# yzhang511/multi_modal_foundation_model

Hardware: AMD Instinct MI355X
Metric: pretrain samples/sec (T=100 bins/modality, d_model=256, 5+5 layers, spike+behaviour masked pretraining step) (higher is better)
Workload: dtype bf16; 1 GPU; BASELINE.json configs[1]: 1 session, ap(668 neurons)+behaviour(2), d_model=256, heads=8, mlp=512, 5 enc + 5 dec layers, T=100 (L=200 tokens), dropout 0.4/0.2, AdamW+OneCycleLR, mixed objectives; per_gpu_batch=1024, global_batch=1024, seq_len=200, parallelism=dp1

## Files before the change

multi_modal_foundation_model_amd/csrc/gemm_bf16.hip:

```cpp
#include "gemm_route.h"
#include <stdlib.h>
#include <algorithm>

namespace {

constexpr int BM = 128, BN = 128;
constexpr int NTHREADS = 256;
template <int BK> struct Geo {
    static constexpr int KC_LD = BK + 8;
    static constexpr int TILE_BYTES = 128 * KC_LD * 2;
    static constexpr int NP = BK / 16;
};

typedef __attribute__((ext_vector_type(8))) __bf16 bf16x8v;
typedef __attribute__((ext_vector_type(4))) short s16x4;
typedef __attribute__((address_space(3))) s16x4 lds_s16x4;

__device__ __forceinline__ uint4 load8(const uint16_t* __restrict__ src, int nvalid, int align) {
    uint4 v = make_uint4(0u, 0u, 0u, 0u);
    if (nvalid >= 8 && align == 8) return *reinterpret_cast<const uint4*>(src);
    if (nvalid >= 8 && align == 4) {
        const uint2 a = *reinterpret_cast<const uint2*>(src), b = *reinterpret_cast<const uint2*>(src + 4);
        return make_uint4(a.x, a.y, b.x, b.y);
    }
    if (nvalid <= 0) return v;
    uint16_t e[8];
#pragma unroll
    for (int j = 0; j < 8; ++j) e[j] = (j < nvalid) ? src[j] : (uint16_t)0;
    v.x = e[0] | ((uint32_t)e[1] << 16); v.y = e[2] | ((uint32_t)e[3] << 16);
    v.z = e[4] | ((uint32_t)e[5] << 16); v.w = e[6] | ((uint32_t)e[7] << 16);
    return v;
}

template <bool RC, int BK>
__device__ __forceinline__ void g2r(uint4 (&r)[BK / 16], const uint16_t* __restrict__ base, int ld, int row0, int k0, int rows, int kend,
                                    int align, int t) {
    constexpr int NP = BK / 16, LPR = BK / 8, RPP = 256 / LPR;
    if (!RC) {
        const int kq = t % LPR, r0 = t / LPR, k = k0 + 8 * kq;
#pragma unroll
        for (int p = 0; p < NP; ++p) {
            const int row = row0 + r0 + RPP * p;
            r[p] = (row < rows) ? load8(base + (size_t)row * ld + k, kend - k, align) : make_uint4(0u, 0u, 0u, 0u);
        }
    } else {
        const int cq = t & 15, kk0 = t >> 4, col = row0 + 8 * cq;
#pragma unroll
        for (int p = 0; p < NP; ++p) {
            const int k = k0 + kk0 + 16 * p;
            r[p] = (k < kend) ? load8(base + (size_t)k * ld + col, rows - col, align) : make_uint4(0u, 0u, 0u, 0u);
        }
    }
}

template <bool RC, int BK>
__device__ __forceinline__ void r2s(char* __restrict__ S, const uint4 (&r)[BK / 16], int t) {
    constexpr int NP = BK / 16, LPR = BK / 8, RPP = 256 / LPR, KC_LD = Geo<BK>::KC_LD;
    if (!RC) {
        const int kq = t % LPR, r0 = t / LPR;
#pragma unroll
        for (int p = 0; p < NP; ++p) *reinterpret_cast<uint4*>(S + (r0 + RPP * p) * (KC_LD * 2) + kq * 16) = r[p];
    } else {
        const int cq = t & 15, kk0 = t >> 4;
#pragma unroll
        for (int p = 0; p < NP; ++p) {
            const int kk = kk0 + 16 * p;
            *reinterpret_cast<uint4*>(S + kk * 256 + ((cq * 16) ^ ((kk & 3) << 6))) = r[p];
        }
    }
}

template <bool RC, int BK>
__device__ __forceinline__ bf16x8v frag(const char* __restrict__ S, int rowbase, int ks, int lane) {
    if (!RC) {
        const int r = lane & 31, h = lane >> 5;
        const uint4 v = *reinterpret_cast<const uint4*>(S + (rowbase + r) * (Geo<BK>::KC_LD * 2) + ks * 32 + h * 16);
        return __builtin_bit_cast(bf16x8v, v);
    } else {
        const int g = lane >> 4, li = lane & 15, q = li >> 2, p = li & 3;
        const int col = rowbase + 16 * (g & 1) + 4 * p;
        const int kb = ks * 16 + 8 * (g >> 1);
        const int off0 = (kb + q) * 256 + ((col * 2) ^ (q << 6));
        const int off1 = (kb + 4 + q) * 256 + ((col * 2) ^ (q << 6));
        const s16x4 lo = __builtin_amdgcn_ds_read_tr16_b64_v4i16((lds_s16x4*)(S + off0));
        const s16x4 hi = __builtin_amdgcn_ds_read_tr16_b64_v4i16((lds_s16x4*)(S + off1));
        typedef __attribute__((ext_vector_type(8))) short s16x8;
        s16x8 v;
        v[0] = lo[0]; v[1] = lo[1]; v[2] = lo[2]; v[3] = lo[3]; v[4] = hi[0]; v[5] = hi[1]; v[6] = hi[2]; v[7] = hi[3];
        return __builtin_bit_cast(bf16x8v, v);
    }
}

template <typename TO, int AK = 0, int EF = 0>
__device__ __forceinline__ void epilogue_store(const mmfm_gemm_desc& d, const LiveArg& lv, const Drop& dr, float v, int m, int n) {
    typedef io<uint16_t> I16;
    constexpr int AKM = AK == kActEmbed ? 0 : AK;
    if (d.bias) v += d.bias[n];
    if (d.pre_out) I16::st(reinterpret_cast<uint16_t*>(d.pre_out) + (size_t)m * d.ldc + n, v);
    if constexpr (AK == kActEmbed) {
        if (!(d.act & 1)) v = embed_act1<true, EF>(v) * d.act_scale;
        else if (EF == 0) v *= d.act_scale;
        else v = embed_mul_grad1<true, EF>(v, I16::ld(reinterpret_cast<const uint16_t*>(d.gradmul_pre) + (size_t)m * d.ldc + n)) * d.act_scale;
        if (dr.on()) v = dr.apply(v, (uint64_t)live_orig_row(lv, m) * (uint64_t)d.N + (uint64_t)n);
        if (d.residual) v += I16::ld(reinterpret_cast<const uint16_t*>(d.residual) + (size_t)m * d.ldr + n);
        io<TO>::st(reinterpret_cast<TO*>(d.C) + (size_t)m * d.ldc + n, v);
        return;
    }
    if (d.act == 1) v = gelu_poly(v);
    else if (d.act == 2) v = softsign_f(v) * d.act_scale;
    else if (AK && !(d.act & 1)) v = mlp_act1<AKM>(v, d.act_scale);
    if (d.gradmul_pre) {
        const float u = I16::ld(reinterpret_cast<const uint16_t*>(d.gradmul_pre) + (size_t)m * d.ldc + n);
        if (AK == MMFM_MLP_RELU) v = u > 0.f ? v : 0.f;
        else if (AK) v *= mlp_act_grad1<AKM>(u, d.act_scale);
        else v *= (d.act == 3) ? gelu_poly_grad(u) : (d.act == 4 ? softsign_grad(u) : softsign_grad_from_out(u, 1.f / d.act_scale)) * d.act_scale;
    }
    if (dr.on()) v = dr.apply(v, (uint64_t)live_orig_row(lv, m) * (uint64_t)d.N + (uint64_t)n);
    if (d.residual) v += I16::ld(reinterpret_cast<const uint16_t*>(d.residual) + (size_t)m * d.ldr + n);
    io<TO>::st(reinterpret_cast<TO*>(d.C) + (size_t)m * d.ldc + n, v);
}

typedef __attribute__((ext_vector_type(8))) __bf16 bf16x8e;
__device__ __forceinline__ bf16x8e pack8f(const float* v) {
    bf16x8e o;
#pragma unroll
    for (int e = 0; e < 8; ++e) o[e] = (__bf16)v[e];
    return o;
}
__device__ __forceinline__ void unpack8(uint4 w, float* u) {
    u[0] = __uint_as_float(w.x << 16); u[1] = __uint_as_float(w.x & 0xffff0000u);
    u[2] = __uint_as_float(w.y << 16); u[3] = __uint_as_float(w.y & 0xffff0000u);
    u[4] = __uint_as_float(w.z << 16); u[5] = __uint_as_float(w.z & 0xffff0000u);
    u[6] = __uint_as_float(w.w << 16); u[7] = __uint_as_float(w.w & 0xffff0000u);
}

__device__ __forceinline__ int xcd_remap(int bid, int nwg) {
    const int q = nwg >> 3, r = nwg & 7, x = bid & 7;
    return (x < r ? x * (q + 1) : r * (q + 1) + (x - r) * q) + (bid >> 3);
}

__device__ __forceinline__ uint4 ldg8(const uint16_t* p, bool a16, bool hi, bool nt) {
    if (a16 && nt) return __builtin_bit_cast(uint4, __builtin_nontemporal_load(reinterpret_cast<const mmfm_u32x4*>(p)));
    if (a16) return *reinterpret_cast<const uint4*>(p);
    const uint2 a = *reinterpret_cast<const uint2*>(p);
    const uint2 b = hi ? *reinterpret_cast<const uint2*>(p + 4) : make_uint2(0u, 0u);
    return make_uint4(a.x, a.y, b.x, b.y);
}
__device__ __forceinline__ void stg8(uint16_t* p, uint4 v, bool a16, bool hi, bool nt) {
    if (nt) {
        if (a16) { st_stream(reinterpret_cast<uint4*>(p), v); return; }
        st_stream(reinterpret_cast<uint2*>(p), make_uint2(v.x, v.y));
        if (hi) st_stream(reinterpret_cast<uint2*>(p + 4), make_uint2(v.z, v.w));
        return;
    }
    if (a16) { *reinterpret_cast<uint4*>(p) = v; return; }
    *reinterpret_cast<uint2*>(p) = make_uint2(v.x, v.y);
    if (hi) *reinterpret_cast<uint2*>(p + 4) = make_uint2(v.z, v.w);
}

template <typename TO, bool EPI_LOADS = true, int AK = 0, int EF = 0>
__device__ __forceinline__ void epilogue_tile(const mmfm_gemm_desc& d, const LiveArg& lv, f32x16 (&acc)[2][2], char* smem, int m0, int n0, int z, int vec_epi,
                                              int t, int wm, int wn, int kh, int l31) {
    const bool split = d.splits > 1;
    constexpr int AKM = AK == kActEmbed ? 0 : AK;
    float* Cf = reinterpret_cast<float*>(d.C) + (split ? (size_t)z * d.slab_stride : 0);
    const Drop dr = drop_init(d.drop);
    if (vec_epi & 1) {
        float* stage = reinterpret_cast<float*>(smem);
        constexpr int SLDW = 132;
        constexpr bool BF_OUT = sizeof(TO) == 2;
        const bool bf_path = BF_OUT && !split;
        const bool a16 = !(vec_epi & 2);
        const int col = (t & 15) * 8, n = n0 + col;
        const bool n_ok = n < d.N, hi = n + 8 <= d.N;
        float bs[8];
#pragma unroll
        for (int e = 0; e < 8; ++e) bs[e] = 0.f;
        if (d.bias && n_ok && !split) {
            const float4 b0 = *reinterpret_cast<const float4*>(d.bias + n);
            const float4 b1 = hi ? *reinterpret_cast<const float4*>(d.bias + n + 4) : make_float4(0.f, 0.f, 0.f, 0.f);
            bs[0] = b0.x; bs[1] = b0.y; bs[2] = b0.z; bs[3] = b0.w; bs[4] = b1.x; bs[5] = b1.y; bs[6] = b1.z; bs[7] = b1.w;
        }
#pragma unroll 1
        for (int half = 0; half < 2; ++half) {
            uint4 gu[4], gr[4];
            if (EPI_LOADS && bf_path) {
#pragma unroll
                for (int c = 0; c < 4; ++c) {
                    const int m = m0 + half * 64 + ((t + 256 * c) >> 4);
                    gu[c] = gr[c] = make_uint4(0u, 0u, 0u, 0u);
                    if (m < d.M && n_ok) {
                        if (d.gradmul_pre) gu[c] = ldg8(reinterpret_cast<const uint16_t*>(d.gradmul_pre) + (size_t)m * d.ldc + n, a16, hi, (vec_epi & 32768) != 0);
                        if (d.residual) gr[c] = ldg8(reinterpret_cast<const uint16_t*>(d.residual) + (size_t)m * d.ldr + n, a16, hi, (vec_epi & 32768) != 0);
                    }
                }
            }
            __syncthreads();
            if (wm == half) {
#pragma unroll
                for (int i = 0; i < 2; ++i)
#pragma unroll
                    for (int j = 0; j < 2; ++j)
#pragma unroll
                        for (int r = 0; r < 16; ++r)
                            stage[(i * 32 + (r & 3) + 8 * (r >> 2) + 4 * kh) * SLDW + wn * 64 + j * 32 + l31] = acc[i][j][r];
            }
            __syncthreads();
#pragma unroll
            for (int c = 0; c < 4; ++c) {
                const int row = (t + 256 * c) >> 4;
                const int m = m0 + half * 64 + row;
                if (m >= d.M || !n_ok) continue;
                float v[8];
                const float4 s0 = *reinterpret_cast<const float4*>(stage + row * SLDW + col);
                const float4 s1 = *reinterpret_cast<const float4*>(stage + row * SLDW + col + 4);
                v[0] = s0.x; v[1] = s0.y; v[2] = s0.z; v[3] = s0.w; v[4] = s1.x; v[5] = s1.y; v[6] = s1.z; v[7] = s1.w;
                const size_t off = (size_t)m * d.ldc + n;
#pragma unroll
                for (int e = 0; e < 8; ++e) v[e] += bs[e];
                if (split || !BF_OUT) {
                    float* dst = (split ? Cf : reinterpret_cast<float*>(d.C)) + off;
                    if (vec_epi & 16384) {
                        st_stream(reinterpret_cast<float4*>(dst), make_float4(v[0], v[1], v[2], v[3]));
                        if (hi) st_stream(reinterpret_cast<float4*>(dst + 4), make_float4(v[4], v[5], v[6], v[7]));
                    } else {
                        *reinterpret_cast<float4*>(dst) = make_float4(v[0], v[1], v[2], v[3]);
                        if (hi) *reinterpret_cast<float4*>(dst + 4) = make_float4(v[4], v[5], v[6], v[7]);
                    }
                    continue;
                }
                if (d.pre_out) stg8(reinterpret_cast<uint16_t*>(d.pre_out) + off, __builtin_bit_cast(uint4, pack8f(v)), a16, hi, (vec_epi & 8192) != 0);
                if constexpr (AK == kActEmbed) {
                    if (!(d.act & 1)) embed_act_n<8, EF>(v, d.act_scale);
                    else {
                        float u[8];
                        unpack8(gu[c], u);
                        embed_mul_grad_n<8, EF>(v, u, d.act_scale);
                    }
                } else if (d.act == 1) gelu_n<8>(v);
                else if (d.act == 2) {
#pragma unroll
                    for (int e = 0; e < 8; ++e) v[e] = softsign_f(v[e]) * d.act_scale;
                } else if (AK && !(d.act & 1)) mlp_act_n<AK, 8>(v, d.act_scale);
                if (AK != kActEmbed && EPI_LOADS && d.gradmul_pre) {
                    float u[8];
                    unpack8(gu[c], u);
                    if (d.act == 3) mul_gelu_grad_n<8>(v, u);
                    else if (d.act == 4) {
#pragma unroll
                        for (int e = 0; e < 8; ++e) v[e] *= softsign_grad(u[e]) * d.act_scale;
                    } else if (AK) mul_mlp_act_grad_n<AKM, 8>(v, u, d.act_scale);
                    else {
                        const float inv_s = 1.f / d.act_scale;
#pragma unroll
                        for (int e = 0; e < 8; ++e) v[e] *= softsign_grad_from_out(u[e], inv_s) * d.act_scale;
                    }
                }
                if (dr.on()) {
                    const uint64_t base = (uint64_t)live_orig_row(lv, m) * (uint64_t)d.N + (uint64_t)n;
#pragma unroll
                    for (int e = 0; e < 8; e += 2) dr.apply2(v[e], v[e + 1], base + e);
                }
                if (EPI_LOADS && d.residual) {
                    float u[8];
                    unpack8(gr[c], u);
#pragma unroll
                    for (int e = 0; e < 8; ++e) v[e] += u[e];
                }
                stg8(reinterpret_cast<uint16_t*>(d.C) + off, __builtin_bit_cast(uint4, pack8f(v)), a16, hi, (vec_epi & 4096) != 0);
            }
        }
        return;
    }
    if (split) {
#pragma unroll
        for (int i = 0; i < 2; ++i)
#pragma unroll
            for (int j = 0; j < 2; ++j)
#pragma unroll
                for (int r = 0; r < 16; ++r) {
                    const int m = m0 + wm * 64 + i * 32 + (r & 3) + 8 * (r >> 2) + 4 * kh;
                    const int n = n0 + wn * 64 + j * 32 + l31;
                    if (m < d.M && n < d.N) Cf[(size_t)m * d.ldc + n] = acc[i][j][r];
                }
        return;
    }
#pragma unroll
    for (int i = 0; i < 2; ++i)
#pragma unroll
        for (int j = 0; j < 2; ++j)
#pragma unroll
            for (int r = 0; r < 16; ++r) {
                const int m = m0 + wm * 64 + i * 32 + (r & 3) + 8 * (r >> 2) + 4 * kh;
                const int n = n0 + wn * 64 + j * 32 + l31;
                if (m < d.M && n < d.N) epilogue_store<TO, AK, EF>(d, lv, dr, acc[i][j][r], m, n);
            }
}

template <bool ARC, bool BRC, typename TO, int BK, bool PERSIST = (sizeof(TO) == 4), int AK = 0>
__global__ __launch_bounds__(NTHREADS, BK == 64 ? 3 : 2) void gemm_bf16_kernel(const mmfm_gemm_desc d_full, const int alignA, const int alignB,
                                                                              const int vec_epi, const int items_full, const LiveArg lv) {
    mmfm_gemm_desc d = d_full;
    live_patch(d, lv);
    const int total_items = (lv.rec && !lv.kdim) ? ((d.M + BM - 1) / BM) * ((d.N + BN - 1) / BN) : items_full;
    constexpr int TILE_BYTES = Geo<BK>::TILE_BYTES;
    __shared__ __attribute__((aligned(16))) char smem[2 * TILE_BYTES];
    char* As = smem;
    char* Bs = smem + TILE_BYTES;
    const int t = threadIdx.x, lane = t & 63, wave = t >> 6;
    const int wm = wave >> 1, wn = wave & 1, kh = lane >> 5, l31 = lane & 31;
    const int tiles_n = (d.N + BN - 1) / BN;
    const int tiles = ((d.M + BM - 1) / BM) * tiles_n;
    const uint16_t* A = reinterpret_cast<const uint16_t*>(d.A);
    const uint16_t* B = reinterpret_cast<const uint16_t*>(d.B);

    auto decode = [&](int w, int& m0, int& n0, int& z, int& kbeg, int& kend) {
        const int item = xcd_remap(w, total_items);
        z = item / tiles;
        const int tile = item - z * tiles;
        m0 = (tile / tiles_n) * BM;
        n0 = (tile % tiles_n) * BN;
        kbeg = z * d.kchunk;
        kend = min(d.K, kbeg + d.kchunk);
    };

    int m0, n0, z, kbeg, kend;
    int w = blockIdx.x;
    if (w >= total_items) return;
    decode(w, m0, n0, z, kbeg, kend);
    uint4 ra[BK / 16], rb[BK / 16];
    g2r<ARC, BK>(ra, A, d.lda, m0, kbeg, d.M, kend, alignA, t);
    g2r<BRC, BK>(rb, B, d.ldb, n0, kbeg, d.N, kend, alignB, t);
    for (;;) {
        f32x16 acc[2][2];
#pragma unroll
        for (int i = 0; i < 2; ++i)
#pragma unroll
            for (int j = 0; j < 2; ++j)
#pragma unroll
                for (int r = 0; r < 16; ++r) acc[i][j][r] = 0.f;
        const bool do_cs = ARC && d.colsum != nullptr && n0 == 0;
        float cs[8];
#pragma unroll
        for (int j = 0; j < 8; ++j) cs[j] = 0.f;
        const int wn_ = w + gridDim.x;
        const bool more = PERSIST && wn_ < total_items;
        int m0n = 0, n0n = 0, zn = 0, kbegn = 0, kendn = 0;
        if (more) decode(wn_, m0n, n0n, zn, kbegn, kendn);
        for (int k0 = kbeg; k0 < kend; k0 += BK) {
            __syncthreads();
            r2s<ARC, BK>(As, ra, t);
            r2s<BRC, BK>(Bs, rb, t);
            __syncthreads();
            {
                if (k0 + BK < kend) {
                    g2r<ARC, BK>(ra, A, d.lda, m0, k0 + BK, d.M, kend, alignA, t);
                    g2r<BRC, BK>(rb, B, d.ldb, n0, k0 + BK, d.N, kend, alignB, t);
                } else if (more) {
                    g2r<ARC, BK>(ra, A, d.lda, m0n, kbegn, d.M, kendn, alignA, t);
                    g2r<BRC, BK>(rb, B, d.ldb, n0n, kbegn, d.N, kendn, alignB, t);
                }
            }
            if (ARC && do_cs) {
                const int cq = t & 15, kk0 = t >> 4;
#pragma unroll
                for (int p = 0; p < BK / 16; ++p) {
                    const int kk = kk0 + 16 * p;
                    float u[8];
                    unpack8(*reinterpret_cast<const uint4*>(As + kk * 256 + ((cq * 16) ^ ((kk & 3) << 6))), u);
#pragma unroll
                    for (int j = 0; j < 8; ++j) cs[j] += u[j];
                }
            }
#pragma unroll
            for (int ks = 0; ks < BK / 16; ++ks) {
                const bf16x8v a0 = frag<ARC, BK>(As, wm * 64, ks, lane), a1 = frag<ARC, BK>(As, wm * 64 + 32, ks, lane);
                const bf16x8v b0 = frag<BRC, BK>(Bs, wn * 64, ks, lane), b1 = frag<BRC, BK>(Bs, wn * 64 + 32, ks, lane);
                acc[0][0] = __builtin_amdgcn_mfma_f32_32x32x16_bf16(a0, b0, acc[0][0], 0, 0, 0);
                acc[0][1] = __builtin_amdgcn_mfma_f32_32x32x16_bf16(a0, b1, acc[0][1], 0, 0, 0);
                acc[1][0] = __builtin_amdgcn_mfma_f32_32x32x16_bf16(a1, b0, acc[1][0], 0, 0, 0);
                acc[1][1] = __builtin_amdgcn_mfma_f32_32x32x16_bf16(a1, b1, acc[1][1], 0, 0, 0);
            }
        }
        if (ARC && do_cs) {
            __syncthreads();
            float* red = reinterpret_cast<float*>(smem);
            float* mine = red + (t >> 4) * 128 + (t & 15) * 8;
            *reinterpret_cast<float4*>(mine) = make_float4(cs[0], cs[1], cs[2], cs[3]);
            *reinterpret_cast<float4*>(mine + 4) = make_float4(cs[4], cs[5], cs[6], cs[7]);
            __syncthreads();
            if (t < 128 && m0 + t < d.M) {
                float sum = 0.f;
#pragma unroll
                for (int i = 0; i < 16; ++i) sum += red[i * 128 + t];
                d.colsum[(d.splits > 1 ? (size_t)z * d.slab_stride : 0) + m0 + t] = sum;
            }
        }
        if constexpr (AK == kActEmbed)
            embed_dispatch(d.act, [&](auto F) {
                epilogue_tile<TO, !(PERSIST && sizeof(TO) == 2), AK, decltype(F)::value>(d, lv, acc, smem, m0, n0, z, vec_epi, t, wm, wn, kh, l31);
            });
        else
            epilogue_tile<TO, !(PERSIST && sizeof(TO) == 2), AK>(d, lv, acc, smem, m0, n0, z, vec_epi, t, wm, wn, kh, l31);
        if (!more) break;
        w = wn_; m0 = m0n; n0 = n0n; z = zn; kbeg = kbegn; kend = kendn;
    }
}

int align_of(const void* p, int ld) {
    if (gemm_ld8(ld) && gemm_al16(p)) return 8;
    if (ld % 4 == 0 && (uintptr_t)p % 8 == 0) return 4;
    return 1;
}

}

int mmfm_gemm_bf16_launch(const mmfm_gemm_desc& d, hipStream_t st, const LiveArg& lv) {
    static const int bk_env = [] { const char* e = getenv("MMFM_GEMM_BK"); return e ? atoi(e) : 0; }();
    const int BKsel = bk_env == 128 ? 128 : 64;
    const int tiles = cdiv(d.M, BM) * cdiv(d.N, BN);
    const int aA = align_of(d.A, d.lda), aB = align_of(d.B, d.ldb);
    const int total_items = tiles * d.splits;
    static const int wg_per_cu = [] { const char* e = getenv("MMFM_GEMM_WG_PER_CU"); const int v = e ? atoi(e) : 3; return v > 0 ? v : 3; }();
    const bool f32out = d.c_f32 || d.splits > 1;
    const auto al16 = gemm_al16;
    const int vec8 = (d.N % 8 == 0) && gemm_ld8(d.ldc) && al16(d.C) && al16(d.pre_out) && al16(d.gradmul_pre) && al16(d.bias) &&
                     (!d.residual || (gemm_ld8(d.ldr) && al16(d.residual))) && (!d.splits || d.splits == 1 || d.slab_stride % 4 == 0);
    auto al8 = [](const void* p) { return p == nullptr || (uintptr_t)p % 8 == 0; };
    const bool f32c = d.c_f32 || d.splits > 1;
    const int vec4 = (d.N % 4 == 0) && (d.ldc % 4 == 0) && (f32c ? al16(d.C) : al8(d.C)) && al8(d.pre_out) && al8(d.gradmul_pre) && al16(d.bias) &&
                     (!d.residual || (d.ldr % 4 == 0 && al8(d.residual))) && (!d.splits || d.splits == 1 || d.slab_stride % 4 == 0);
    const int vec = vec8 ? 1 : (vec4 ? 3 : 0);
    static const int nt_env = [] { const char* e = getenv("MMFM_GEMM_NT"); return e ? atoi(e) : 3; }();
    const int vecf = vec | ((nt_env & 1) ? 4096 : 0) | ((nt_env & 2) ? 8192 : 0) | ((nt_env & 4) ? 16384 : 0) | ((nt_env & 8) ? 32768 : 0);
    static const int persist_bf16 = [] { const char* e = getenv("MMFM_GEMM_PERSIST_BF16"); return e ? atoi(e) : 1; }();
    const int ak = gemm_act_kind(d.act);
    const bool pb = !f32out && !ak && persist_bf16 && !d.gradmul_pre && !d.residual && !d.pre_out && (vec & 1) && d.K <= 768;
    dim3 grid((f32out || pb) ? std::min(total_items, 256 * wg_per_cu) : total_items), block(NTHREADS);
    static const int pad_lds = [] { const char* e = getenv("MMFM_GEMM_PAD_LDS"); return e ? atoi(e) : 0; }();
#define LAUNCH2(ARC, BRC, BKV)                                                                                    \
    if (f32out) hipLaunchKernelGGL((gemm_bf16_kernel<ARC, BRC, float, BKV>), grid, block, pad_lds, st, d, aA, aB, vecf, total_items, lv);  \
    else if (pb) hipLaunchKernelGGL((gemm_bf16_kernel<ARC, BRC, uint16_t, BKV, true>), grid, block, pad_lds, st, d, aA, aB, vecf, total_items, lv); \
    else hipLaunchKernelGGL((gemm_bf16_kernel<ARC, BRC, uint16_t, BKV>), grid, block, pad_lds, st, d, aA, aB, vecf, total_items, lv);
#define LAUNCH_AK(ARC, BRC, AKV)                                                                                  \
    if (f32out) hipLaunchKernelGGL((gemm_bf16_kernel<ARC, BRC, float, 64, true, AKV>), grid, block, pad_lds, st, d, aA, aB, vecf, total_items, lv); \
    else hipLaunchKernelGGL((gemm_bf16_kernel<ARC, BRC, uint16_t, 64, false, AKV>), grid, block, pad_lds, st, d, aA, aB, vecf, total_items, lv);
#define LAUNCH(ARC, BRC)                                                                                          \
    if (ak == MMFM_MLP_RELU) { LAUNCH_AK(ARC, BRC, MMFM_MLP_RELU) }                                                \
    else if (ak == MMFM_MLP_SIGMOID) { LAUNCH_AK(ARC, BRC, MMFM_MLP_SIGMOID) }                                     \
    else if (ak == MMFM_MLP_GELU_TANH) { LAUNCH_AK(ARC, BRC, MMFM_MLP_GELU_TANH) }                                 \
    else if (ak == kActEmbed) { LAUNCH_AK(ARC, BRC, kActEmbed) }                                                   \
    else if (BKsel == 128) { LAUNCH2(ARC, BRC, 128) } else { LAUNCH2(ARC, BRC, 64) }
    if (d.a_kcontig && d.b_kcontig) { LAUNCH(false, false) }
    else if (d.a_kcontig && !d.b_kcontig) { LAUNCH(false, true) }
    else { LAUNCH(true, true) }
#undef LAUNCH
#undef LAUNCH_AK
#undef LAUNCH2
    MMFM_LAUNCH_CHECK("mmfm_gemm(bf16)");
    return 0;
}
```

multi_modal_foundation_model_amd/csrc/gemm_route.h:

```cpp
#pragma once
#include "common.h"

struct GemmRoute {
    int family = 0;
};

inline bool gemm_al16(const void* p) { return p == nullptr || (uintptr_t)p % 16 == 0; }
inline bool gemm_ld8(int ld) { return ld % 8 == 0; }

bool mmfm_gemm_big_takes(const mmfm_gemm_desc& d, const LiveArg& lv);
int mmfm_gemm_big_launch(const mmfm_gemm_desc& d, hipStream_t st, const LiveArg& lv);
bool mmfm_gemm_dw_takes(const mmfm_gemm_desc& d, const LiveArg& lv, bool& wide);
bool mmfm_gemm_dw_pair_takes(const mmfm_gemm_desc& a, const mmfm_gemm_desc& b);
int mmfm_gemm_dw_launch(const mmfm_gemm_desc& d, const mmfm_gemm_desc* second, bool wide, hipStream_t st, const LiveArg& lv);
int mmfm_gemm_bf16_launch(const mmfm_gemm_desc& d, hipStream_t st, const LiveArg& lv);

int mmfm_gemm_routed(const mmfm_gemm_desc& d, hipStream_t st);
```

Before: 37100 samples/s.

## Route thin-dimension GEMMs to dedicated small-K and thin weight-gradient kernels

```diff
diff --git a/multi_modal_foundation_model_amd/csrc/gemm_bf16.hip b/multi_modal_foundation_model_amd/csrc/gemm_bf16.hip
--- a/multi_modal_foundation_model_amd/csrc/gemm_bf16.hip
+++ b/multi_modal_foundation_model_amd/csrc/gemm_bf16.hip
@@ -1,4 +1,5 @@
 #include "gemm_route.h"
+#include "gemm_epilogue.h"
 #include <stdlib.h>
 #include <algorithm>
 
@@ -91,49 +92,6 @@
     }
 }
 
-template <typename TO, int AK = 0, int EF = 0>
-__device__ __forceinline__ void epilogue_store(const mmfm_gemm_desc& d, const LiveArg& lv, const Drop& dr, float v, int m, int n) {
-    typedef io<uint16_t> I16;
-    constexpr int AKM = AK == kActEmbed ? 0 : AK;
-    if (d.bias) v += d.bias[n];
-    if (d.pre_out) I16::st(reinterpret_cast<uint16_t*>(d.pre_out) + (size_t)m * d.ldc + n, v);
-    if constexpr (AK == kActEmbed) {
-        if (!(d.act & 1)) v = embed_act1<true, EF>(v) * d.act_scale;
-        else if (EF == 0) v *= d.act_scale;
-        else v = embed_mul_grad1<true, EF>(v, I16::ld(reinterpret_cast<const uint16_t*>(d.gradmul_pre) + (size_t)m * d.ldc + n)) * d.act_scale;
-        if (dr.on()) v = dr.apply(v, (uint64_t)live_orig_row(lv, m) * (uint64_t)d.N + (uint64_t)n);
-        if (d.residual) v += I16::ld(reinterpret_cast<const uint16_t*>(d.residual) + (size_t)m * d.ldr + n);
-        io<TO>::st(reinterpret_cast<TO*>(d.C) + (size_t)m * d.ldc + n, v);
-        return;
-    }
-    if (d.act == 1) v = gelu_poly(v);
-    else if (d.act == 2) v = softsign_f(v) * d.act_scale;
-    else if (AK && !(d.act & 1)) v = mlp_act1<AKM>(v, d.act_scale);
-    if (d.gradmul_pre) {
-        const float u = I16::ld(reinterpret_cast<const uint16_t*>(d.gradmul_pre) + (size_t)m * d.ldc + n);
-        if (AK == MMFM_MLP_RELU) v = u > 0.f ? v : 0.f;
-        else if (AK) v *= mlp_act_grad1<AKM>(u, d.act_scale);
-        else v *= (d.act == 3) ? gelu_poly_grad(u) : (d.act == 4 ? softsign_grad(u) : softsign_grad_from_out(u, 1.f / d.act_scale)) * d.act_scale;
-    }
-    if (dr.on()) v = dr.apply(v, (uint64_t)live_orig_row(lv, m) * (uint64_t)d.N + (uint64_t)n);
-    if (d.residual) v += I16::ld(reinterpret_cast<const uint16_t*>(d.residual) + (size_t)m * d.ldr + n);
-    io<TO>::st(reinterpret_cast<TO*>(d.C) + (size_t)m * d.ldc + n, v);
-}
-
-typedef __attribute__((ext_vector_type(8))) __bf16 bf16x8e;
-__device__ __forceinline__ bf16x8e pack8f(const float* v) {
-    bf16x8e o;
-#pragma unroll
-    for (int e = 0; e < 8; ++e) o[e] = (__bf16)v[e];
-    return o;
-}
-__device__ __forceinline__ void unpack8(uint4 w, float* u) {
-    u[0] = __uint_as_float(w.x << 16); u[1] = __uint_as_float(w.x & 0xffff0000u);
-    u[2] = __uint_as_float(w.y << 16); u[3] = __uint_as_float(w.y & 0xffff0000u);
-    u[4] = __uint_as_float(w.z << 16); u[5] = __uint_as_float(w.z & 0xffff0000u);
-    u[6] = __uint_as_float(w.w << 16); u[7] = __uint_as_float(w.w & 0xffff0000u);
-}
-
 __device__ __forceinline__ int xcd_remap(int bid, int nwg) {
     const int q = nwg >> 3, r = nwg & 7, x = bid & 7;
     return (x < r ? x * (q + 1) : r * (q + 1) + (x - r) * q) + (bid >> 3);
@@ -416,6 +374,7 @@
 }
 
 int mmfm_gemm_bf16_launch(const mmfm_gemm_desc& d, hipStream_t st, const LiveArg& lv) {
+    if (mmfm_gemm_thin_takes(d, lv)) return mmfm_gemm_thin_launch(d, st, lv);
     static const int bk_env = [] { const char* e = getenv("MMFM_GEMM_BK"); return e ? atoi(e) : 0; }();
     const int BKsel = bk_env == 128 ? 128 : 64;
     const int tiles = cdiv(d.M, BM) * cdiv(d.N, BN);
diff --git a/multi_modal_foundation_model_amd/csrc/gemm_epilogue.h b/multi_modal_foundation_model_amd/csrc/gemm_epilogue.h
--- /dev/null
+++ b/multi_modal_foundation_model_amd/csrc/gemm_epilogue.h
@@ -0,0 +1,76 @@
+#pragma once
+#include "common.h"
+
+typedef __attribute__((ext_vector_type(8))) __bf16 bf16x8e;
+__device__ __forceinline__ bf16x8e pack8f(const float* v) {
+    bf16x8e o;
+#pragma unroll
+    for (int e = 0; e < 8; ++e) o[e] = (__bf16)v[e];
+    return o;
+}
+__device__ __forceinline__ void unpack8(uint4 w, float* u) {
+    u[0] = __uint_as_float(w.x << 16); u[1] = __uint_as_float(w.x & 0xffff0000u);
+    u[2] = __uint_as_float(w.y << 16); u[3] = __uint_as_float(w.y & 0xffff0000u);
+    u[4] = __uint_as_float(w.z << 16); u[5] = __uint_as_float(w.z & 0xffff0000u);
+    u[6] = __uint_as_float(w.w << 16); u[7] = __uint_as_float(w.w & 0xffff0000u);
+}
+
+template <int AK = 0, int EF = 0, int NV = 1>
+__device__ __forceinline__ void epilogue_values(const mmfm_gemm_desc& d, const LiveArg& lv, const Drop& dr, float (&v)[NV], int m, int n) {
+    typedef io<uint16_t> I16;
+    constexpr int AKM = AK == kActEmbed ? 0 : AK;
+    const size_t oc = (size_t)m * d.ldc + n;
+    if (d.bias) {
+#pragma unroll
+        for (int e = 0; e < NV; ++e) v[e] += d.bias[n + e];
+    }
+    if (d.pre_out) {
+#pragma unroll
+        for (int e = 0; e < NV; ++e) I16::st(reinterpret_cast<uint16_t*>(d.pre_out) + oc + e, v[e]);
+    }
+    if constexpr (AK == kActEmbed) {
+#pragma unroll
+        for (int e = 0; e < NV; ++e) {
+            if (!(d.act & 1)) v[e] = embed_act1<true, EF>(v[e]) * d.act_scale;
+            else if (EF == 0) v[e] *= d.act_scale;
+            else v[e] = embed_mul_grad1<true, EF>(v[e], I16::ld(reinterpret_cast<const uint16_t*>(d.gradmul_pre) + oc + e)) * d.act_scale;
+        }
+    } else {
+#pragma unroll
+        for (int e = 0; e < NV; ++e) {
+            if (d.act == 1) v[e] = gelu_poly(v[e]);
+            else if (d.act == 2) v[e] = softsign_f(v[e]) * d.act_scale;
+            else if (AK && !(d.act & 1)) v[e] = mlp_act1<AKM>(v[e], d.act_scale);
+        }
+        if (d.gradmul_pre) {
+#pragma unroll
+            for (int e = 0; e < NV; ++e) {
+                const float u = I16::ld(reinterpret_cast<const uint16_t*>(d.gradmul_pre) + oc + e);
+                if (AK == MMFM_MLP_RELU) v[e] = u > 0.f ? v[e] : 0.f;
+                else if (AK) v[e] *= mlp_act_grad1<AKM>(u, d.act_scale);
+                else v[e] *= (d.act == 3) ? gelu_poly_grad(u) : (d.act == 4 ? softsign_grad(u) : softsign_grad_from_out(u, 1.f / d.act_scale)) * d.act_scale;
+            }
+        }
+    }
+    if (dr.on()) {
+        const uint64_t base = (uint64_t)live_orig_row(lv, m) * (uint64_t)d.N + (uint64_t)n;
+        if constexpr (NV % 2 == 0) {
+#pragma unroll
+            for (int e = 0; e < NV; e += 2) dr.apply2(v[e], v[e + 1], base + e);
+        } else {
+#pragma unroll
+            for (int e = 0; e < NV; ++e) v[e] = dr.apply(v[e], base + e);
+        }
+    }
+    if (d.residual) {
+#pragma unroll
+        for (int e = 0; e < NV; ++e) v[e] += I16::ld(reinterpret_cast<const uint16_t*>(d.residual) + (size_t)m * d.ldr + n + e);
+    }
+}
+
+template <typename TO, int AK = 0, int EF = 0>
+__device__ __forceinline__ void epilogue_store(const mmfm_gemm_desc& d, const LiveArg& lv, const Drop& dr, float v, int m, int n) {
+    float a[1] = {v};
+    epilogue_values<AK, EF, 1>(d, lv, dr, a, m, n);
+    io<TO>::st(reinterpret_cast<TO*>(d.C) + (size_t)m * d.ldc + n, a[0]);
+}
diff --git a/multi_modal_foundation_model_amd/csrc/gemm_route.h b/multi_modal_foundation_model_amd/csrc/gemm_route.h
--- a/multi_modal_foundation_model_amd/csrc/gemm_route.h
+++ b/multi_modal_foundation_model_amd/csrc/gemm_route.h
@@ -14,5 +14,7 @@
 bool mmfm_gemm_dw_pair_takes(const mmfm_gemm_desc& a, const mmfm_gemm_desc& b);
 int mmfm_gemm_dw_launch(const mmfm_gemm_desc& d, const mmfm_gemm_desc* second, bool wide, hipStream_t st, const LiveArg& lv);
 int mmfm_gemm_bf16_launch(const mmfm_gemm_desc& d, hipStream_t st, const LiveArg& lv);
+bool mmfm_gemm_thin_takes(const mmfm_gemm_desc& d, const LiveArg& lv);
+int mmfm_gemm_thin_launch(const mmfm_gemm_desc& d, hipStream_t st, const LiveArg& lv);
 
 int mmfm_gemm_routed(const mmfm_gemm_desc& d, hipStream_t st);
diff --git a/multi_modal_foundation_model_amd/csrc/gemm_thin.hip b/multi_modal_foundation_model_amd/csrc/gemm_thin.hip
--- /dev/null
+++ b/multi_modal_foundation_model_amd/csrc/gemm_thin.hip
@@ -0,0 +1,244 @@
+#include "gemm_route.h"
+#include "gemm_epilogue.h"
+#include <stdlib.h>
+
+namespace {
+
+constexpr int kThin = 8;
+constexpr int kWide = 2048;
+constexpr int FWD_THREADS = 256, KROWS = 4;
+constexpr int DW_THREADS = 1024, DW_UNROLL = 8;
+
+__device__ __forceinline__ void ld_thin(const uint16_t* __restrict__ p, int n, bool vec, float (&f)[8]) {
+    uint4 w = make_uint4(0u, 0u, 0u, 0u);
+    if (vec && n == 8) w = *reinterpret_cast<const uint4*>(p);
+    else if (vec && n == 4) { const uint2 a = *reinterpret_cast<const uint2*>(p); w.x = a.x; w.y = a.y; }
+    else if (vec && n == 2) w.x = *reinterpret_cast<const uint32_t*>(p);
+    else {
+        uint16_t e[8];
+#pragma unroll
+        for (int j = 0; j < 8; ++j) e[j] = (j < n) ? p[j] : (uint16_t)0;
+        w.x = e[0] | ((uint32_t)e[1] << 16); w.y = e[2] | ((uint32_t)e[3] << 16);
+        w.z = e[4] | ((uint32_t)e[5] << 16); w.w = e[6] | ((uint32_t)e[7] << 16);
+    }
+    unpack8(w, f);
+}
+template <int VW> __device__ __forceinline__ void ld_wide(const uint16_t* __restrict__ p, float (&f)[VW]) {
+    if constexpr (VW == 8) {
+        unpack8(*reinterpret_cast<const uint4*>(p), f);
+    } else if constexpr (VW == 4) {
+        const uint2 a = *reinterpret_cast<const uint2*>(p);
+        f[0] = __uint_as_float(a.x << 16); f[1] = __uint_as_float(a.x & 0xffff0000u);
+        f[2] = __uint_as_float(a.y << 16); f[3] = __uint_as_float(a.y & 0xffff0000u);
+    } else if constexpr (VW == 2) {
+        const uint32_t a = *reinterpret_cast<const uint32_t*>(p);
+        f[0] = __uint_as_float(a << 16); f[1] = __uint_as_float(a & 0xffff0000u);
+    } else {
+        f[0] = bf2f(*p);
+    }
+}
+
+__device__ __forceinline__ void stage_w(uint16_t* Ws, const mmfm_gemm_desc& d, int ldw, int t, int nthreads) {
+    const uint16_t* B = reinterpret_cast<const uint16_t*>(d.B);
+    const int total = d.N * d.K;
+    for (int i = t; i < total; i += nthreads) {
+        int n, k;
+        if (d.b_kcontig) { n = i / d.K; k = i - n * d.K; } else { k = i / d.N; n = i - k * d.N; }
+        const uint16_t w = d.b_kcontig ? B[(size_t)n * d.ldb + k] : B[(size_t)k * d.ldb + n];
+        Ws[k * ldw + n] = w;
+    }
+}
+
+template <int CH>
+__global__ __launch_bounds__(FWD_THREADS) void thin_k_kernel(const mmfm_gemm_desc d_full, const int avec, const int cshift, const LiveArg lv) {
+    extern __shared__ __attribute__((aligned(16))) uint16_t Ws[];
+    mmfm_gemm_desc d = d_full;
+    live_patch(d, lv);
+    const int t = threadIdx.x, cpr = d.N / CH, ldw = (d.N + 7) & ~7;
+    const int items = d.M * cpr, i0 = blockIdx.x * (KROWS * FWD_THREADS) + t;
+    if (i0 - t >= items) return;
+    auto row_of = [&](int i) { return cshift >= 0 ? i >> cshift : i / cpr; };
+    stage_w(Ws, d, ldw, t, FWD_THREADS);
+    const uint16_t* A = reinterpret_cast<const uint16_t*>(d.A);
+    float a[KROWS][8];
+#pragma unroll
+    for (int r = 0; r < KROWS; ++r) {
+        const int i = i0 + r * FWD_THREADS;
+#pragma unroll
+        for (int k = 0; k < 8; ++k) a[r][k] = 0.f;
+        if (i < items) ld_thin(A + (size_t)row_of(i) * d.lda, d.K, avec != 0, a[r]);
+    }
+    __syncthreads();
+    const Drop dr = drop_init(d.drop);
+#pragma unroll
+    for (int r = 0; r < KROWS; ++r) {
+        const int i = i0 + r * FWD_THREADS;
+        if (i >= items) continue;
+        const int m = row_of(i), n = (i - m * cpr) * CH;
+        float acc[CH];
+#pragma unroll
+        for (int e = 0; e < CH; ++e) acc[e] = 0.f;
+#pragma unroll
+        for (int k = 0; k < 8; ++k) {
+            if (k >= d.K) break;
+            float w[CH];
+            if constexpr (CH == 1) w[0] = bf2f(Ws[k * ldw + n]);
+            else ld_wide<CH>(Ws + k * ldw + n, w);
+#pragma unroll
+            for (int e = 0; e < CH; ++e) acc[e] = fmaf(a[r][k], w[e], acc[e]);
+        }
+        epilogue_values<0, 0, CH>(d, lv, dr, acc, m, n);
+        uint16_t* c = reinterpret_cast<uint16_t*>(d.C) + (size_t)m * d.ldc + n;
+        if constexpr (CH == 8) *reinterpret_cast<uint4*>(c) = __builtin_bit_cast(uint4, pack8f(acc));
+        else if constexpr (CH == 4) io<uint16_t>::st4(c, make_float4(acc[0], acc[1], acc[2], acc[3]));
+        else io<uint16_t>::st(c, acc[0]);
+    }
+}
+
+template <int VW, bool AWIDE>
+__global__ __launch_bounds__(DW_THREADS) void thin_dw_kernel(const mmfm_gemm_desc d_full, const int CT, const int RL, const int qvec, const LiveArg lv) {
+    constexpr int TM = 8 / VW, CSN = AWIDE ? VW : TM, SLOTS = 8 + CSN;
+    __shared__ float red[SLOTS * DW_THREADS];
+    mmfm_gemm_desc d = d_full;
+    live_patch(d, lv);
+    const int z = blockIdx.x, t = threadIdx.x, ct = t % CT, rl = t / CT;
+    const bool active = rl < RL;
+    const int kbeg = (int)min((int64_t)z * d.kchunk, (int64_t)d.K), kend = (int)min((int64_t)d.K, (int64_t)kbeg + d.kchunk);
+    const int T = AWIDE ? d.N : d.M, w0 = ct * VW;
+    const uint16_t* P = reinterpret_cast<const uint16_t*>(AWIDE ? d.A : d.B) + w0;
+    const uint16_t* Q = reinterpret_cast<const uint16_t*>(AWIDE ? d.B : d.A);
+    const int ldp = AWIDE ? d.lda : d.ldb, ldq = AWIDE ? d.ldb : d.lda;
+    float acc[VW][TM], cs[CSN];
+#pragma unroll
+    for (int i = 0; i < VW; ++i)
+#pragma unroll
+        for (int jn = 0; jn < TM; ++jn) acc[i][jn] = 0.f;
+#pragma unroll
+    for (int i = 0; i < CSN; ++i) cs[i] = 0.f;
+    if (active) {
+        for (int k0 = kbeg + rl; k0 < kend; k0 += RL * DW_UNROLL) {
+            float p[DW_UNROLL][VW], q[DW_UNROLL][8];
+#pragma unroll
+            for (int u = 0; u < DW_UNROLL; ++u) {
+                const int k = k0 + u * RL;
+#pragma unroll
+                for (int i = 0; i < VW; ++i) p[u][i] = 0.f;
+#pragma unroll
+                for (int i = 0; i < 8; ++i) q[u][i] = 0.f;
+                if (k < kend) {
+                    ld_wide<VW>(P + (size_t)k * ldp, p[u]);
+                    ld_thin(Q + (size_t)k * ldq, T, qvec != 0, q[u]);
+                }
+            }
+#pragma unroll
+            for (int u = 0; u < DW_UNROLL; ++u) {
+#pragma unroll
+                for (int i = 0; i < VW; ++i)
+#pragma unroll
+                    for (int jn = 0; jn < TM; ++jn) acc[i][jn] = fmaf(p[u][i], q[u][jn], acc[i][jn]);
+#pragma unroll
+                for (int i = 0; i < CSN; ++i) cs[i] += AWIDE ? p[u][i] : q[u][i];
+            }
+        }
+#pragma unroll
+        for (int i = 0; i < VW; ++i)
+#pragma unroll
+            for (int jn = 0; jn < TM; ++jn) red[(i * TM + jn) * DW_THREADS + t] = acc[i][jn];
+#pragma unroll
+        for (int i = 0; i < CSN; ++i) red[(8 + i) * DW_THREADS + t] = cs[i];
+    }
+    for (int h = RL >> 1; h > 0; h >>= 1) {
+        __syncthreads();
+        if (rl < h) {
+#pragma unroll
+            for (int s = 0; s < SLOTS; ++s) red[s * DW_THREADS + t] += red[s * DW_THREADS + t + h * CT];
+        }
+    }
+    if (rl != 0) return;
+    const size_t slab = d.splits > 1 ? (size_t)z * d.slab_stride : 0;
+    float* C = reinterpret_cast<float*>(d.C) + slab;
+#pragma unroll
+    for (int i = 0; i < VW; ++i)
+#pragma unroll
+        for (int jn = 0; jn < TM; ++jn) {
+            if (jn >= T) continue;
+            const float v = red[(i * TM + jn) * DW_THREADS + t];
+            if (AWIDE) C[(size_t)(w0 + i) * d.ldc + jn] = v; else C[(size_t)jn * d.ldc + w0 + i] = v;
+        }
+    if (d.colsum) {
+#pragma unroll
+        for (int i = 0; i < CSN; ++i) {
+            const float v = red[(8 + i) * DW_THREADS + t];
+            if (AWIDE) d.colsum[slab + w0 + i] = v;
+            else if (ct == 0 && i < T) d.colsum[slab + i] = v;
+        }
+    }
+}
+
+bool al_to(const void* p, int bytes) { return (uintptr_t)p % bytes == 0; }
+
+enum { THIN_NONE = 0, THIN_K, THIN_DW };
+
+bool dw_geometry(const mmfm_gemm_desc& d, bool& awide, int& VW, int& CT, int& RL) {
+    awide = d.M >= d.N;
+    const int W = awide ? d.M : d.N, T = awide ? d.N : d.M, ldp = awide ? d.lda : d.ldb;
+    const void* P = awide ? d.A : d.B;
+    if (W > kThin) return false;
+    VW = T == 1 ? 8 : (T == 2 ? 4 : (T <= 4 ? 2 : 1));
+    while (VW > 1 && !(W % VW == 0 && ldp % VW == 0 && al_to(P, 2 * VW))) VW >>= 1;
+    CT = W / VW;
+    RL = 1;
+    while (CT * RL * 2 <= DW_THREADS) RL *= 2;
+    return true;
+}
+
+int thin_class(const mmfm_gemm_desc& d) {
+    static const int on = [] { const char* e = getenv("MMFM_GEMM_THIN"); return e ? atoi(e) : 1; }();
+    if (!on || d.dtype != MMFM_BF16) return THIN_NONE;
+    if (d.M > kThin && d.N > kThin && d.K > kThin) return THIN_NONE;
+    const bool plain_epi = !d.bias && !d.pre_out && !d.act && !d.gradmul_pre && !d.residual && d.drop.p <= 0.f;
+    if (!d.a_kcontig && !d.b_kcontig) {
+        bool awide; int VW, CT, RL;
+        if (!(d.c_f32 || d.splits > 1) || !plain_epi || !al_to(d.C, 4)) return THIN_NONE;
+        return dw_geometry(d, awide, VW, CT, RL) ? THIN_DW : THIN_NONE;
+    }
+    if (!d.a_kcontig) return THIN_NONE;
+    if (d.c_f32 || d.splits > 1 || d.colsum || gemm_act_kind(d.act) || d.pre_out || d.residual) return THIN_NONE;
+    return (d.K <= kThin && d.N <= kWide && (int64_t)d.M * d.N < (1ll << 30)) ? THIN_K : THIN_NONE;
+}
+
+}
+
+bool mmfm_gemm_thin_takes(const mmfm_gemm_desc& d, const LiveArg& lv) { return thin_class(d) != THIN_NONE; }
+
+int mmfm_gemm_thin_launch(const mmfm_gemm_desc& d, hipStream_t st, const LiveArg& lv) {
+    const int cls = thin_class(d);
+    if (cls == THIN_K) {
+        auto al8 = [](const void* p) { return p == nullptr || (uintptr_t)p % 8 == 0; };
+        const bool vec8 = d.N % 8 == 0 && gemm_ld8(d.ldc) && gemm_al16(d.C) && gemm_al16(d.gradmul_pre) && gemm_al16(d.bias);
+        const bool vec4 = d.N % 4 == 0 && d.ldc % 4 == 0 && al8(d.C) && al8(d.gradmul_pre) && gemm_al16(d.bias);
+        const int CH = vec8 ? 8 : (vec4 ? 4 : 1);
+        const int avec = (d.K == 2 || d.K == 4 || d.K == 8) && d.lda % d.K == 0 && al_to(d.A, 2 * d.K);
+        const int cpr = d.N / CH, cshift = (cpr & (cpr - 1)) == 0 ? __builtin_ctz(cpr) : -1;
+        const dim3 grid(cdiv((long)d.M * cpr, KROWS * FWD_THREADS)), block(FWD_THREADS);
+        const size_t lds = (size_t)d.K * ((d.N + 7) & ~7) * 2;
+        if (CH == 8) hipLaunchKernelGGL(thin_k_kernel<8>, grid, block, lds, st, d, avec, cshift, lv);
+        else if (CH == 4) hipLaunchKernelGGL(thin_k_kernel<4>, grid, block, lds, st, d, avec, cshift, lv);
+        else hipLaunchKernelGGL(thin_k_kernel<1>, grid, block, lds, st, d, avec, cshift, lv);
+    } else if (cls == THIN_DW) {
+        bool awide; int VW, CT, RL;
+        dw_geometry(d, awide, VW, CT, RL);
+        const int T = awide ? d.N : d.M, ldq = awide ? d.ldb : d.lda;
+        const int qvec = (T == 2 || T == 4 || T == 8) && ldq % T == 0 && al_to(awide ? d.B : d.A, 2 * T);
+        const dim3 grid(d.splits), block(DW_THREADS);
+#define THIN_DW_LAUNCH(V)                                                                                          \
+        if (awide) hipLaunchKernelGGL((thin_dw_kernel<V, true>), grid, block, 0, st, d, CT, RL, qvec, lv);        \
+        else hipLaunchKernelGGL((thin_dw_kernel<V, false>), grid, block, 0, st, d, CT, RL, qvec, lv);
+        if (VW == 8) { THIN_DW_LAUNCH(8) } else if (VW == 4) { THIN_DW_LAUNCH(4) } else if (VW == 2) { THIN_DW_LAUNCH(2) } else { THIN_DW_LAUNCH(1) }
+#undef THIN_DW_LAUNCH
+    } else {
+        return mmfm_set_error(-1, "mmfm_gemm(thin): descriptor not taken");
+    }
+    MMFM_LAUNCH_CHECK("mmfm_gemm(thin)");
+    return 0;
+}
```

After: 37290 samples/s, median of 6. About the same (+0.5%).
